# angelocatalani/neural-network-compression

Measured on AMD Instinct MI355X. Metric: weights/sec through prune+k-means (K=256), higher is better.
Workload: dtype f32

## Files before the change

### neural_network_compression_amd/csrc/nnc_hip.hip

```cpp
#include "nnc_common.hpp"
#include "nnc_km_shared.hpp"


extern "C" size_t nnc_kmeans_workspace_bytes(int32_t k)
{
    (void)k;
    return sizeof(KmWs) + 256;
}

extern "C" int32_t nnc_fix_shift(float absmax, int64_t n_total)
{
    int L = 1;
    while (((int64_t)1 << L) < n_total && L < 62) L++;
    if (!(absmax > 0.0f) || !std::isfinite(absmax)) return 0;
    int P = 0;
    (void)std::frexp((double)absmax, &P);
    return std::min(28, 62 - L) - P;
}

__device__ __forceinline__ int fix_f32(float v, int Sft)
{
    return (int)rintf(ldexpf(v, Sft));
}

// ... 1097 lines not shown
    return *word;
}

template <int NT, bool MASS>
__device__ int km_finalize_relocate(KmWs *__restrict__ ws, const float *__restrict__ xs, const long long n, const KmTab *__restrict__ tab, const int ku,
                                    const int k, const int cur, long long *sum_o, long long *cnt_o, const float mean, const int Sft)
{
    constexpr int KC = NNC_KMAX;
    __shared__ __align__(16) unsigned char buf[sizeof(KlHead) + (size_t)KC * (8 + 8 + 4 + 4 + 4 + 4 + 2 + 2) + 4096 * 2];
    KlHead *hd = reinterpret_cast<KlHead *>(buf);
    KlArr L = {};
    {
        unsigned char *q = buf + sizeof(KlHead);
        L.A = reinterpret_cast<long long *>(q); q += (size_t)KC * 8;
        L.B = reinterpret_cast<long long *>(q); q += (size_t)KC * 8;
        L.cs = reinterpret_cast<float *>(q); q += (size_t)KC * 4;
        L.csq = reinterpret_cast<float *>(q); q += (size_t)KC * 4;
        L.cold = reinterpret_cast<float *>(q); q += (size_t)KC * 4;
        L.call = reinterpret_cast<float *>(q); q += (size_t)KC * 4;
        L.so = reinterpret_cast<uint16_t *>(q); q += (size_t)KC * 2;
        L.phi = reinterpret_cast<uint16_t *>(q); q += (size_t)KC * 2;
        L.qj = reinterpret_cast<uint16_t *>(q);
    }
    const int tid = threadIdx.x;
    if (tid == 0) { hd->n_empty = 0; hd->ku = ku; hd->nch = 0; hd->slow = 0; hd->r_flat = 0; }
    __syncthreads();
    int e = 0;
    for (int j = tid; j < k; j += NT) { e += cnt_o[j] == 0; L.cold[j] = ws->c[cur][j]; }
    if (e) atomicAdd(&hd->n_empty, e);
    __syncthreads();
    const bool mass = MASS && hd->n_empty > KL_RM_MAX;
    if (!MASS && hd->n_empty > KL_RM_MAX) return 0;
    if (!mass && 2 * ku > KL_RPASS * (NT / 8)) return 0;
    for (int p = tid; p < ku; p += NT) {
        const float2 c = tab->cand[p];
        L.cs[p] = c.x; L.csq[p] = c.y; L.so[p] = tab->orig[p];
        L.A[p] = ws->hint_a[p]; L.B[p] = ws->hint_b[p];
        const int ph = ws->bnd_phi[p];
        L.phi[p] = (uint16_t)(ph < p + 1 ? p + 1 : (ph > ku - 1 ? ku - 1 : ph));
    }
    __syncthreads();
    int *qfirst = reinterpret_cast<int *>(L.call);
    for (int j = tid; j + 1 < ku; j += NT) {
        const long long bm = j > 0 ? L.B[j - 1] : 0, a = L.A[j], b = L.B[j];
        const long long s0 = a > bm ? a : bm;
        const long long len = b - s0;
        qfirst[j] = 0;
        if (len > 0) {
            const int cs_ = (int)L.phi[j] == j + 1 ? KL_CHUNK : KL_CHUNK_CROWD;
            const long long nc = (len + cs_ - 1) / cs_;
            if (nc > (mass ? 512 : 64)) hd->slow = 1;
            else {
                const int first = atomicAdd(&hd->nch, (int)nc);
                qfirst[j] = first;
                for (int i = 0; i < (int)nc; i++) if (first + i < KL_QMAX) L.qj[first + i] = (uint16_t)j;
            }
        }
    }
    __syncthreads();
    if (NNC_FIN_TRACE_PTR && tid == 0) {
        unsigned long long *rt = NNC_FIN_TRACE_PTR;
        const int it = min(ws->st.iter, 63);
        rt[300 + 4 * it] = (unsigned long long)hd->n_empty; rt[301 + 4 * it] = (unsigned long long)hd->nch; rt[302 + 4 * it] = (unsigned long long)hd->slow; rt[303 + 4 * it] = (unsigned long long)ku;
    }
    if (hd->slow || hd->nch > 1024) return 0;
    if constexpr (MASS) {
        if (mass) {
            __shared__ KlMass mass_s;
            return kl_relocate_mass<NT>(xs, n, ws, hd, L, &mass_s, sum_o, cnt_o, k, hd->nch, mean, Sft);
        }
    }
    return kl_relocate<NT>(xs, n, ws, hd, L, sum_o, cnt_o, k, hd->nch, mean, Sft);
}

template <int NT, bool ONEWAVE, bool MASS = false>
__device__ __forceinline__ bool km_finalize_body(KmWs *__restrict__ ws, int mode, int resume, int *gcell, int *hcell, int *ku_out, const bool lazy = false,
                                                 const float *__restrict__ reloc_xs = nullptr, const long long reloc_n = 0, const int k_hint = 0)
{
    static_assert(!ONEWAVE || NT == 64, "the barrier-free form is for a single wave");
#define FIN_SYNC() do { if (ONEWAVE) wave_lds_fence(); else km_lds_barrier(); } while (0)
#define FIN_OR(slot, x) (ONEWAVE ? (int)__any(x) : km_vote_or(&fin_votes[slot], (x)))
#define FIN_AND(slot, x) (ONEWAVE ? (int)__all(x) : !km_vote_or(&fin_votes[slot], !(x)))
#define FIN_COUNT(slot, x) (ONEWAVE ? (int)__popcll(__ballot(x)) : km_vote_count(&fin_votes[slot], (x)))
    __shared__ int fin_votes[8];
    __shared__ long long sum_o[NNC_KMAX];
    __shared__ long long cnt_o[NNC_KMAX];
    __shared__ __align__(16) float cnew[NNC_KMAX];
    __shared__ float cs[NNC_KMAX];
    __shared__ uint16_t so[NNC_KMAX];
    __shared__ float sq[NNC_KMAX];
    __shared__ unsigned long long sh_key;
    __shared__ int ovf_n;
    __shared__ PwHeap heap;
    __shared__ float cu[NNC_KMAX];
    __shared__ uint16_t sou[NNC_KMAX];
    __shared__ double wave_a[NT / 64], wave_b[NT / 64];

    const int tid = threadIdx.x;
    unsigned long long *ftr = NNC_FIN_TRACE_PTR;
#define FSTAMP(i) do { if (ftr && tid == 0) ftr[i] = __builtin_amdgcn_s_memrealtime(); } while (0)
    FSTAMP(0);
    if (tid == 0) ws->cells_pending = 0;
    if (!ONEWAVE && tid < 8) fin_votes[tid] = 0;
    const int kb = k_hint > 0 ? min(k_hint, (int)NNC_KMAX) : (int)NNC_KMAX;
    const bool takes_a_pass = mode != FIN_FROM_PARTIALS;
    const bool from_shards = mode == FIN_FROM_SHARDS || mode == FIN_PACK_ONLY;
    const int qn_raw = takes_a_pass ? ws->q_n : 0;
    const int st_done = ws->st.done, st_paused = ws->st.paused, st_iter = ws->st.iter, reloc_fail = ws->reloc_fail;
    const int spec_go = ws->spec_go;
    const int k = ws->p.k, Sft = ws->p.fix_shift, max_iter = ws->p.max_iter, glog2 = ws->glog2;
    const float tol_v = ws->p.tol, p_lo = ws->p.lo, p_hi = ws->p.hi, inv_f = ws->inv;
    const long long n_tot = ws->p.n_total;
    const int ku0 = ws->tab[0].ku, ku1 = ws->tab[1].ku;
    int cur = ws->cur;
    const bool track = (mode == FIN_FROM_SHARDS) || (mode == FIN_FROM_PARTIALS && !resume);
    constexpr int RR = 2;
    long long pc[RR];
    float c_both[RR][2];
    uint16_t pm_both[RR][2], pmn_both[RR][2];
#pragma unroll
    for (int r = 0; r < RR; r++) {
        pc[r] = 0; c_both[r][0] = c_both[r][1] = 0.0f; pm_both[r][0] = pm_both[r][1] = pmn_both[r][0] = pmn_both[r][1] = 0;
        const int j = tid + r * NT;
        if (j < kb) {
            if (track) pc[r] = ws->prev_counts[j];
            if (mode != FIN_INIT) {
                c_both[r][0] = ws->c[0][j]; c_both[r][1] = ws->c[1][j];
                pm_both[r][0] = ws->tab[0].perm[j]; pm_both[r][1] = ws->tab[1].perm[j];
                if (j + 1 < NNC_KMAX) { pmn_both[r][0] = ws->tab[0].perm[j + 1]; pmn_both[r][1] = ws->tab[1].perm[j + 1]; }
            }
        }
    }
    long long sh_s[KM_NSHARD];
    unsigned long long sh_c[KM_NSHARD];
    uint16_t og_both[2] = {0, 0};
    const bool sh_pre = from_shards && tid < kb;
#pragma unroll
    for (int sh = 0; sh < KM_NSHARD; sh++) { sh_s[sh] = 0; sh_c[sh] = 0; }
    if (sh_pre) {
        og_both[0] = ws->tab[0].orig[tid]; og_both[1] = ws->tab[1].orig[tid];
#pragma unroll
        for (int sh = 0; sh < KM_NSHARD; sh++) { sh_s[sh] = ws->shard_sum[sh][tid]; sh_c[sh] = ws->shard_cnt[sh][tid]; }
    }
    const int qn = min(qn_raw, (int)NNC_KMAX);
    for (int r = tid; r < qn; r += NT) { ws->q_w0[r] = 0ull; ws->q_w1[r] = 0ull; ws->q_next[r] = 0; }
    FSTAMP(44);
#define FIN_QUEUE_RESET() do { if (tid == 0 && takes_a_pass) { ws->q_n = 0; ws->q_searched = 0; ws->help_hint = qn > 0; } } while (0)
#define FIN_LEAVE() do { if (ONEWAVE) wave_lds_fence(); else __syncthreads(); FIN_QUEUE_RESET(); return false; } while (0)
    if (mode != FIN_INIT && mode != FIN_PACK_ONLY && st_done) FIN_LEAVE();
    if (mode == FIN_FROM_SHARDS && st_paused) FIN_LEAVE();
    if (mode == FIN_PACK_ONLY && (st_done | st_paused)) {
        const int k2 = 2 * k;
        for (int i = tid; i < k2; i += NT) ws->partials[i] = ws->partials_local[i];
        FIN_LEAVE();
    }
    if (mode == FIN_FROM_PARTIALS && st_paused && !resume) FIN_LEAVE();
    if (resume == 2 && !spec_go) FIN_LEAVE();
    if (resume && reloc_fail) {
        if (tid == 0) ws->st.paused = 2;
        FIN_LEAVE();
    }

    float cold_r[RR];
    int spa[RR], spb[RR];
#pragma unroll
    for (int r = 0; r < RR; r++) {
        const int j = tid + r * NT;
        const bool in = mode != FIN_INIT && j < k;
        cold_r[r] = in ? (cur ? c_both[r][1] : c_both[r][0]) : 0.0f;
        spa[r] = in ? (int)(cur ? pm_both[r][1] : pm_both[r][0]) : 0;
        spb[r] = (in && j + 1 < k) ? (int)(cur ? pmn_both[r][1] : pmn_both[r][0]) : 0;
        if (!(track && j < k)) pc[r] = 0;
    }
    if (from_shards) {
        const KmTab *tab = &ws->tab[cur];
        const int ku_cur = cur ? ku1 : ku0;
        for (int j = tid; j < k; j += NT) { sum_o[j] = 0; cnt_o[j] = 0; }
        FIN_SYNC();
        FIN_QUEUE_RESET();
        FSTAMP(45);
        for (int p = tid; p < ku_cur; p += NT) {
            long long s = 0;
            unsigned long long c = 0;
            int o;
            if (p == tid && sh_pre) {
                o = cur ? og_both[1] : og_both[0];
#pragma unroll
                for (int sh = 0; sh < KM_NSHARD; sh++) { s += sh_s[sh]; c += sh_c[sh]; }
            } else {
                o = tab->orig[p];
                for (int sh = 0; sh < KM_NSHARD; sh++) { s += ws->shard_sum[sh][p]; c += ws->shard_cnt[sh][p]; }
            }
            for (int sh = 0; sh < KM_NSHARD; sh++) { ws->shard_sum[sh][p] = 0; ws->shard_cnt[sh][p] = 0; }
            sum_o[o] = s; cnt_o[o] = (long long)c;
        }
        FIN_SYNC();
        FSTAMP(46);
        for (int j = tid; j < k; j += NT) {
            ws->partials[j] = sum_o[j]; ws->partials[k + j] = cnt_o[j];
            ws->partials_local[j] = sum_o[j]; ws->partials_local[k + j] = cnt_o[j];
        }
        if (mode == FIN_PACK_ONLY) return false;
    } else if (mode == FIN_FROM_PARTIALS) {
        for (int j = tid; j < k; j += NT) { sum_o[j] = ws->partials[j]; cnt_o[j] = ws->partials[k + j]; }
    }
    FIN_SYNC();
    FSTAMP(47);
    if (!from_shards) FIN_QUEUE_RESET();
    int same_counts_now = 0;
    bool settled_event = false;
    if (track) {
        int count_diff = 0;
#pragma unroll
        for (int r = 0; r < RR; r++) {
            const int j = tid + r * NT;
            if (j < k) {
                const long long c = cnt_o[j];
                count_diff |= (pc[r] != c);
                ws->prev_counts[j] = c;
            }
        }
        const int any_diff = FIN_OR(0, count_diff);
        same_counts_now = any_diff ? 0 : 1;
        if (tid == 0) ws->st.same_counts = any_diff ? 0 : 1;
    }
    FSTAMP(1);

    if (mode != FIN_INIT) {
        int my_empty = 0;
        for (int j = tid; j < k; j += NT) my_empty += (cnt_o[j] == 0);
        if (tid == 0) sh_key = 0ull;
        int n_empty = FIN_COUNT(1, my_empty);
        bool settled = false;
        settled_event = false;
        if constexpr (!ONEWAVE) {
            if (n_empty > 0 && (MASS || n_empty <= KL_RM_MAX) && !resume && reloc_xs && mode == FIN_FROM_SHARDS && lazy && !(st_iter >= 1 && same_counts_now)) {
                __syncthreads();
                if (ftr && tid == 0) { ftr[20] = ftr[0]; ftr[21] = __builtin_amdgcn_s_memrealtime(); }
                const KmTab *tabc = &ws->tab[cur];
                settled = km_finalize_relocate<NT, MASS>(ws, reloc_xs, reloc_n, tabc, cur ? ku1 : ku0, k, cur, sum_o, cnt_o, ws->p.x_mean, Sft) != 0;
                if (settled) { n_empty = 0; settled_event = true; }
                if (settled && ftr && tid == 0) ftr[22] = __builtin_amdgcn_s_memrealtime();
            }
        }
        if (n_empty > 0 && !resume) {
            int tot_empty = 0;
            if (tid == 0) {
                for (int j = 0; j < k; j++) tot_empty += (cnt_o[j] == 0);
                ws->st.paused = 1; ws->st.n_empty = tot_empty;
                if (lazy) ws->tab[cur].n_ovf = 0;
            }
            return false;
        }
        for (int j = tid; j < k; j += NT)
            if (cnt_o[j] > 0) cnew[j] = (float)ldexp((double)sum_o[j] / (double)cnt_o[j], -Sft);
        FIN_SYNC();
        if (n_empty > 0) {
            for (int j = tid; j < k; j += NT)
                atomicMax(&sh_key, ((unsigned long long)cnt_o[j] << 11) | (unsigned long long)(2047 - j));
            FIN_SYNC();
            const int amax = 2047 - (int)(sh_key & 2047ull);
            for (int j = tid; j < k; j += NT)
                if (cnt_o[j] <= 0) {
                    cnew[j] = (amax < j) ? cnew[amax] : (float)ldexp((double)sum_o[amax], -Sft);
                }
            FIN_SYNC();
        }
        FSTAMP(2);
#pragma unroll
        for (int r = 0; r < RR; r++) {
            const int j = tid + r * NT;
            if (j < k) {
                float d = cnew[j] - cold_r[r];
                float s2 = d * d;
                float sft = (float)sqrt((double)s2);
                sq[j] = sft * sft;
            }
        }
        FIN_SYNC();
        float tot = 0.0f;
        if (ONEWAVE) tot = block_pairwise_sum<true>([&](int i) { return sq[i]; }, k, &heap);
        else if (tid < 64) tot = wave_pairwise_sum([&](int i) { return sq[i]; }, k, &heap);
        if (tid == 0) {
            int iter = st_iter + 1;
            int done = 0;
            if (tot <= tol_v) done = 1;
            else if (iter >= max_iter) done = 2;
            ws->st.iter = iter; ws->st.shift_tot = tot; ws->st.done = done;
            ws->st.paused = 0; ws->st.n_empty = 0;
            ws->cur = cur ^ 1;
        }
        cur ^= 1;
        for (int j = tid; j < k; j += NT) ws->c[cur][j] = cnew[j];
        FIN_SYNC();
    } else {
        for (int j = tid; j < k; j += NT) cnew[j] = ws->c[cur][j];
        FIN_SYNC();
    }

    FSTAMP(3);
    KmTab *tab = &ws->tab[cur];
    int still_sorted = 0;
    if (mode != FIN_INIT) {
        int ok = 1;
#pragma unroll
        for (int r = 0; r < RR; r++) {
            const int p = tid + r * NT;
            if (p < k) {
                const int a = spa[r];
                so[p] = (uint16_t)a;
                cs[p] = cnew[a];
                if (p + 1 < k) {
                    const int b = spb[r];
                    const float va = cnew[a], vb = cnew[b];
                    ok &= (va < vb) || (va == vb && a < b);
                }
            }
        }
        FSTAMP(12);
        still_sorted = FIN_AND(2, ok);
        const bool moved_far = resume || settled_event;
        for (int pass = 0; pass < 3 && !still_sorted && !moved_far; pass++) {
            for (int parity = 0; parity < 2; parity++) {
                for (int p = 2 * tid + parity; p + 1 < k; p += 2 * NT) {
                    const float va = cs[p], vb = cs[p + 1];
                    const uint16_t a = so[p], b = so[p + 1];
                    if (!((va < vb) || (va == vb && a < b))) { cs[p] = vb; cs[p + 1] = va; so[p] = b; so[p + 1] = a; }
                }
                FIN_SYNC();
            }
            int ok2 = 1;
            for (int p = tid; p + 1 < k; p += NT) {
                const float va = cs[p], vb = cs[p + 1];
                ok2 &= (va < vb) || (va == vb && so[p] < so[p + 1]);
            }
            still_sorted = FIN_AND(3 + pass, ok2);
        }
    }
    FSTAMP(8);
    if (ftr && tid == 0) ftr[13] = (unsigned long long)still_sorted;
    if (!still_sorted) {
        int parts = 1;
        while (parts < 64 && k * parts * 2 <= NT) parts <<= 1;
        const int per_part = (((k + parts - 1) / parts) + 3) & ~3;
        const float4 *c4 = reinterpret_cast<const float4 *>(cnew);
        for (int t = tid; t < ((k * parts + NT - 1) / NT) * NT; t += NT) {
            const int j = t / parts, part = t % parts;
            int rank = 0;
            float v = 0.0f;
            if (j < k) {
                v = cnew[j];
                const int i0 = part * per_part, i1 = min(k, i0 + per_part);
#pragma unroll 4
                for (int i = i0; i < i1; i += 4) {
                    const float4 u = c4[i >> 2];
                    rank += (int)(u.x < v) | ((int)(u.x == v) & (int)(i < j));
                    rank += ((int)(u.y < v) | ((int)(u.y == v) & (int)(i + 1 < j))) & (int)(i + 1 < i1);
                    rank += ((int)(u.z < v) | ((int)(u.z == v) & (int)(i + 2 < j))) & (int)(i + 2 < i1);
                    rank += ((int)(u.w < v) | ((int)(u.w == v) & (int)(i + 3 < j))) & (int)(i + 3 < i1);
                }
            }
            for (int off = 1; off < parts; off <<= 1) rank += __shfl_xor(rank, off);
            if (j < k && part == 0) { cs[rank] = v; so[rank] = (uint16_t)j; }
        }
    }
    FIN_SYNC();
    FSTAMP(9);
    if (settled_event && ftr && tid == 0) { ftr[23] = ftr[3]; ftr[24] = ftr[9]; }
    int ku = 0;
    {
        int *wave_i = reinterpret_cast<int *>(wave_a);
        const int rounds_u = (k + NT - 1) / NT;
        int carry = 0;
        for (int rd = 0; rd < rounds_u; rd++) {
            const int p = rd * NT + tid;
            float v = 0.0f;
            int o = 0, first = 0;
            if (p < k) {
                v = cs[p]; o = so[p];
                tab->perm[p] = (uint16_t)o;
                first = (p == 0) || (cs[p - 1] != v);
            }
            const unsigned long long bal = __ballot(first);
            const int before = __popcll(bal & ((1ull << (tid & 63)) - 1ull));
            if ((tid & 63) == 0) wave_i[tid >> 6] = __popcll(bal);
            FIN_SYNC();
            int pre = carry, tot = carry;
            for (int w = 0; w < NT / 64; w++) { const int wv = wave_i[w]; if (w < (tid >> 6)) pre += wv; tot += wv; }
            if (first) { cu[pre + before] = v; sou[pre + before] = (uint16_t)o; }
            carry = tot;
            FIN_SYNC();
        }
        ku = min(carry, k);
    }
    FSTAMP(10);
    for (int p = tid; p < ku; p += NT) {
        const float v = cu[p];
        cs[p] = v;
        tab->cand[p] = make_float2(v, v * v);
        tab->orig[p] = sou[p];
        ws->bnd.cand[p] = make_float2(v, v * v);
        ws->bnd.orig[p] = sou[p];
    }
    if (tid == 0) { tab->ku = ku; ws->ku_cur = ku; ws->bnd.ku = ku; ovf_n = 0; }
    FIN_SYNC();
    FSTAMP(4);
    const double U = 5.9604644775390625e-08;
    const double xb = fmax(fabs((double)p_lo), fabs((double)p_hi));
    const int G = 1 << glog2;
    const double lo = (double)p_lo;
    const double inv = (double)inv_f;
    const double ra = inv > 0.0 ? (1.0 - 4.0 * U) / inv * (1.0 - 4.0 * U) : 0.0;
    const double rb = inv > 0.0 ? (1.0 + 4.0 * U) / inv * (1.0 + 4.0 * U) : 0.0;
    {
        const int rounds = (ku + NT - 1) / NT;
        int *wave_i = reinterpret_cast<int *>(wave_a);
        int carry_g = -2;
        int wide_zone = 0;
        double *zhi = reinterpret_cast<double *>(sum_o), *zlo = reinterpret_cast<double *>(cnt_o);
        const int zd = ku > 0 ? max(1, min(min(4, NT / max(ku, 1)), NNC_KMAX / max(ku, 1))) : 1;
        for (int t = tid; t < zd * ku; t += NT) {
            const int d = t / ku, p = t - d * ku, q = p + d + 1;
            if (q < ku) {
                const KmZone z = km_pair_zone((double)cs[p], (double)cs[q], xb);
                zhi[d * ku + p] = z.hi; zlo[d * ku + q] = z.lo;
            }
        }
        FSTAMP(13);
        FIN_SYNC();
        FSTAMP(14);
        for (int rd = 0; rd < rounds; rd++) {
            const int p = rd * NT + tid;
            int gp = -2, hp_ = G + 1;
            if (p < ku) {
                const double cp = (double)cs[p];
                double right = p + 1 < ku ? zhi[p] : INFINITY, left = p > 0 ? zlo[p] : -INFINITY;
                for (int q = p + 2; q < ku && q - p <= KM_ZONE_REACH; q++) {
                    const double cq = (double)cs[q];
                    const double mid = 0.5 * (cp + cq);
                    const double delta = cq - cp;
                    if (mid - km_pair_slack(delta, xb) >= right) break;
                    const int d = q - p - 1;
                    if (delta > 0.0) right = fmin(right, d < zd ? zhi[d * ku + p] : km_pair_zone(cp, cq, xb).hi);
                }
                for (int q = p - 2; q >= 0 && p - q <= KM_ZONE_REACH; q--) {
                    const double cq = (double)cs[q];
                    const double mid = 0.5 * (cp + cq);
                    const double delta = cp - cq;
                    if (mid + km_pair_slack(delta, xb) <= left) break;
                    const int d = p - q - 1;
                    if (delta > 0.0) left = fmax(left, d < zd ? zlo[d * ku + p] : km_pair_zone(cq, cp, xb).lo);
// ... 1910 lines not shown
```

### neural_network_compression_amd/csrc/nnc_lloyd.hpp

```cpp

struct KlDiag { unsigned long long ph[16], last, sp[8], slast; };
#ifdef NNC_DIAG
#define KLSTAMP(slot) do { if (threadIdx.x == 0) { const unsigned long long now_ = __builtin_amdgcn_s_memrealtime(); dg->ph[slot] += now_ - dg->last; dg->last = now_; } } while (0)
#define KLSUB(slot) do { if (threadIdx.x == 0) { const unsigned long long now_ = __builtin_amdgcn_s_memrealtime(); dg->sp[slot] += now_ - dg->slast; dg->slast = now_; } } while (0)
#else
#define KLSTAMP(slot) do { } while (0)
#define KLSUB(slot) do { } while (0)
#endif
#define KL_MAXR 24
#define KL_TAIL_MAX 2048

struct KlHeap { int start[64]; int len[64]; float val[64]; };
struct KlHead {
    int ku, slow, nch, n_empty, depth, pad0, pad1, pad2;
    float tot;
    int f_empty, f_diff, f_reorder;
    int wave_i[16];
    double wmax[16], wmin[16];
    KlHeap heap;
    int r_cnt, r_bad, r_flat, r_pad1;
    unsigned long long r_keys[8];
    unsigned long long r_wkey[2][16];
    int r_widx[2][16];
    int r_empty[8], r_old[8];
};
static_assert(sizeof(KlHead) % 16 == 0, "the arrays behind the header are 16-byte aligned");

struct KlArr {
    double *Lb, *Ub;
    long long *sum_s, *cnt_s, *A, *B, *PA, *PB, *prevc, *hint;
    float *hL, *hR, *cs, *csq, *cnew, *cold, *sq, *call, *Lf, *Uf;
    uint16_t *so, *perm, *phi, *qj;
};

static size_t kl_lds_bytes(int kc) { return sizeof(KlHead) + (size_t)kc * (2 * 8 + 9 * 8 + 12 * 4 + 3 * 2) + 4096 * 2; }

__device__ __forceinline__ void kl_carve(unsigned char *smem, int kc, KlHead **hd, KlArr *L)
{
    *hd = reinterpret_cast<KlHead *>(smem);
    unsigned char *p = smem + sizeof(KlHead);
    auto take = [&](size_t bytes) { unsigned char *q = p; p += bytes; return q; };
    L->Lb = reinterpret_cast<double *>(take((size_t)kc * 8)); L->Ub = reinterpret_cast<double *>(take((size_t)kc * 8));
    L->sum_s = reinterpret_cast<long long *>(take((size_t)kc * 8)); L->cnt_s = reinterpret_cast<long long *>(take((size_t)kc * 8));
    L->A = reinterpret_cast<long long *>(take((size_t)kc * 8)); L->B = reinterpret_cast<long long *>(take((size_t)kc * 8));
    L->PA = reinterpret_cast<long long *>(take((size_t)kc * 8)); L->PB = reinterpret_cast<long long *>(take((size_t)kc * 8));
    L->prevc = reinterpret_cast<long long *>(take((size_t)kc * 8)); L->hint = reinterpret_cast<long long *>(take((size_t)kc * 16));
    L->hL = reinterpret_cast<float *>(take((size_t)kc * 8)); L->hR = reinterpret_cast<float *>(take((size_t)kc * 8));
    L->cs = reinterpret_cast<float *>(take((size_t)kc * 4)); L->csq = reinterpret_cast<float *>(take((size_t)kc * 4));
    L->cnew = reinterpret_cast<float *>(take((size_t)kc * 4)); L->cold = reinterpret_cast<float *>(take((size_t)kc * 4));
    L->sq = reinterpret_cast<float *>(take((size_t)kc * 4)); L->call = reinterpret_cast<float *>(take((size_t)kc * 4));
    L->Lf = reinterpret_cast<float *>(take((size_t)kc * 4)); L->Uf = reinterpret_cast<float *>(take((size_t)kc * 4));
    L->so = reinterpret_cast<uint16_t *>(take((size_t)kc * 2)); L->perm = reinterpret_cast<uint16_t *>(take((size_t)kc * 2));
    L->phi = reinterpret_cast<uint16_t *>(take((size_t)kc * 2));
    L->qj = reinterpret_cast<uint16_t *>(take((size_t)4096 * 2));
}

#define KL_DPP_I(v, ctrl) __builtin_amdgcn_update_dpp(0, (v), (ctrl), 0xF, 0xF, true)
#define KL_QP_XOR1 0xB1
#define KL_QP_XOR2 0x4E
#define KL_HALF_MIRROR 0x141
__device__ __forceinline__ int grp8_sum_i(int v)
{
    v += KL_DPP_I(v, KL_QP_XOR1); v += KL_DPP_I(v, KL_QP_XOR2); v += KL_DPP_I(v, KL_HALF_MIRROR);
    return v;
}
__device__ __forceinline__ int grp8_min_i(int v)
{
    v = min(v, KL_DPP_I(v, KL_QP_XOR1)); v = min(v, KL_DPP_I(v, KL_QP_XOR2)); v = min(v, KL_DPP_I(v, KL_HALF_MIRROR));
    return v;
}
__device__ __forceinline__ long long grp8_sum_ll(long long v)
{
#define KL_STEP_LL(ctrl) do { const int lo_ = KL_DPP_I((int)(unsigned)(v & 0xFFFFFFFFll), ctrl), hi_ = KL_DPP_I((int)(v >> 32), ctrl); \
        v += (long long)(((unsigned long long)(unsigned)hi_ << 32) | (unsigned)lo_); } while (0)
    KL_STEP_LL(KL_QP_XOR1); KL_STEP_LL(KL_QP_XOR2); KL_STEP_LL(KL_HALF_MIRROR);
#undef KL_STEP_LL
    return v;
}

__device__ void kl_heap_build(KlHead *hd, int n)
{
    KlHeap *hp = &hd->heap;
    const int lane = threadIdx.x & 63;
    hp->start[lane] = 0; hp->len[lane] = 0; hp->val[lane] = 0.0f;
    wave_lds_fence();
    if (lane == 0) { hp->start[1] = 0; hp->len[1] = n; }
    wave_lds_fence();
    int depth = 0;
    while (depth < 5 && ((n + (1 << depth) - 1) >> depth) > LEAF) depth++;
    if (depth < 5) depth++;
    for (int lev = 0; lev < depth; lev++) {
        const int i = (1 << lev) + lane;
        if (lane < (1 << lev)) {
            const int l = hp->len[i];
            if (l > LEAF) {
                int n2 = l / 2; n2 -= n2 % 8;
                hp->start[2 * i] = hp->start[i]; hp->len[2 * i] = n2;
                hp->start[2 * i + 1] = hp->start[i] + n2; hp->len[2 * i + 1] = l - n2;
            }
        }
        wave_lds_fence();
    }
    if (lane == 0) hd->depth = depth;
}

__device__ __forceinline__ float kl_leaf_sum(const float *e, int st, int l, int j8)
{
// ... 427 lines not shown
            int best = j, besto = 0x7fffffff;
            for (int cc = j; cc <= (int)L.phi[j]; cc++) {
                const float d = L.csq[cc] + (-2.0f * (xc * L.cs[cc]));
                const int oc = (int)L.so[cc];
                if (d < bestd || (d == bestd && oc < besto)) { bestd = d; best = cc; besto = oc; }
            }
            atomicAdd(reinterpret_cast<unsigned long long *>(&L.sum_s[best]), (unsigned long long)((long long)fix_f32(xc, Sft) * len));
            atomicAdd(reinterpret_cast<unsigned long long *>(&L.cnt_s[best]), (unsigned long long)len);
            qfirst[j] = -1;
            hd->r_flat = 1;
        } else if (len > 0) {
            const int cs_ = (int)L.phi[j] == j + 1 ? KL_CHUNK : KL_CHUNK_CROWD;
            const long long nc = (len + cs_ - 1) / cs_;
            if (nc > KL_QONE) hd->slow = 1;
            else {
                const int first = atomicAdd(&hd->nch, (int)nc);
                qfirst[j] = first;
                for (int i = 0; i < (int)nc; i++) if (first + i < KL_QMAX) L.qj[first + i] = (uint16_t)j;
            }
        }
    }
}

template <int NT>
__device__ __forceinline__ void kl_label(const float *__restrict__ xs, const float mean, const int Sft, KlHead *hd, const KlArr &L)
{
    const int tid = threadIdx.x, g = tid >> 3, gl = tid & 7;
    const int nch = hd->nch;
    const int *qfirst = reinterpret_cast<const int *>(L.call);
    for (int c = g; c < nch; c += NT / 8) {
        const int j = (int)L.qj[c];
        const long long bm = j > 0 ? L.B[j - 1] : 0, a = L.A[j], e = L.B[j];
        const long long s = a > bm ? a : bm;
        const int phi = L.phi[j];
        const bool two = phi == j + 1;
        const int cs_ = two ? KL_CHUNK : KL_CHUNK_CROWD;
        const long long start = s + (long long)cs_ * (c - qfirst[j]);
        const long long end = start + cs_ < e ? start + cs_ : e;
        const float c0 = L.cs[j], q0 = L.csq[j], c1 = L.cs[j + 1], q1 = L.csq[j + 1];
        const bool tie1 = L.so[j + 1] < L.so[j];
        long long s0 = 0, s1 = 0;
        int n0 = 0, n1 = 0;
        for (long long r0 = start + gl; r0 < end; r0 += 64) {
            float v[8];
#pragma unroll
            for (int u = 0; u < 8; u++) { const long long r = r0 + 8 * u; v[u] = r < end ? xs[r] : 0.0f; }
#pragma unroll
            for (int u = 0; u < 8; u++) {
                if (r0 + 8 * u < end) {
                    const float xc = v[u] - mean;
                    const int q = fix_f32(xc, Sft);
                    if (two) {
                        const float d0 = q0 + (-2.0f * (xc * c0));
                        const float d1 = q1 + (-2.0f * (xc * c1));
                        if (d1 < d0 || (d1 == d0 && tie1)) { s1 += q; n1++; } else { s0 += q; n0++; }
                    } else {
                        float bestd = q0 + (-2.0f * (xc * c0));
                        int best = j, besto = (int)L.so[j];
                        for (int cc = j + 1; cc <= phi; cc++) {
                            const float d = L.csq[cc] + (-2.0f * (xc * L.cs[cc]));
                            const int oc = (int)L.so[cc];
                            if (d < bestd || (d == bestd && oc < besto)) { bestd = d; best = cc; besto = oc; }
                        }
                        atomicAdd(reinterpret_cast<unsigned long long *>(&L.sum_s[best]), (unsigned long long)(long long)q);
                        atomicAdd(reinterpret_cast<unsigned long long *>(&L.cnt_s[best]), 1ull);
                    }
                }
            }
        }
        const long long S0 = grp8_sum_ll(s0), S1 = grp8_sum_ll(s1);
        const int N01 = grp8_sum_i(n0 | (n1 << 16));
        if (gl == 0) {
            const int N0 = N01 & 0xFFFF, N1 = N01 >> 16;
            if (N0) { atomicAdd(reinterpret_cast<unsigned long long *>(&L.sum_s[j]), (unsigned long long)S0); atomicAdd(reinterpret_cast<unsigned long long *>(&L.cnt_s[j]), (unsigned long long)N0); }
            if (N1) { atomicAdd(reinterpret_cast<unsigned long long *>(&L.sum_s[j + 1]), (unsigned long long)S1); atomicAdd(reinterpret_cast<unsigned long long *>(&L.cnt_s[j + 1]), (unsigned long long)N1); }
        }
    }
}

#define KL_RW 8
#define KL_RM_MAX 7
#define KL_RKPT 16
#define KL_RPASS 10
template <int NT>
__device__ __forceinline__ int kl_relocate(const float *__restrict__ xs, const long long n, KmWs *__restrict__ ws, KlHead *hd, const KlArr &L,
                                           long long *sumo, long long *cnto, const int k, const int nch, const float mean, const int Sft)
{
    const int tid = threadIdx.x, lane = tid & 63, wv = tid >> 6, g = tid >> 3, gl = tid & 7;
    const int ku = hd->ku, m = hd->n_empty;
    if (tid == 0 && m > ws->kl_stats[7]) ws->kl_stats[7] = m;
    if (m < 1 || m > KL_RM_MAX || 2 * ku > KL_RPASS * (NT / 8) || hd->r_flat) { if (tid == 0) ws->kl_stats[6] |= 1; return 0; }
    unsigned long long *keys = ws->kl_keys;
    const int base = 2 * KL_RW * ku;
    unsigned long long *rtr = NNC_FIN_TRACE_PTR;
#define KRSTAMP(i) do { if (rtr && tid == 0) rtr[30 + (i)] = __builtin_amdgcn_s_memrealtime(); } while (0)
    KRSTAMP(0);
    if (tid == 0) { hd->r_cnt = 0; hd->r_bad = 0; }
    __syncthreads();
    unsigned inner = 0u;
    {
        long long rr[KL_RPASS];
        float xq[KL_RPASS];
        bool deep[KL_RPASS];
#pragma unroll
        for (int u = 0; u < KL_RPASS; u++) {
            const int q = g + u * (NT / 8);
            rr[u] = -1; deep[u] = false;
            if (q < 2 * ku) {
                const int p = q >> 1, side = q & 1;
                const long long lo_r = p > 0 ? L.B[p - 1] : 0, hi_r = p == ku - 1 ? n : L.A[p];
                long long r = -1;
                if (side == 0) { r = lo_r + gl; if (r >= hi_r) r = -1; }
                else { r = hi_r - 1 - gl; if (r < lo_r + KL_RW) r = -1; }
                rr[u] = r;
                deep[u] = gl == KL_RW - 1 && hi_r - lo_r > 2 * KL_RW;
            }
        }
#pragma unroll
        for (int u = 0; u < KL_RPASS; u++) xq[u] = rr[u] >= 0 ? xs[rr[u]] : 0.0f;
#pragma unroll
        for (int u = 0; u < KL_RPASS; u++) {
            const int q = g + u * (NT / 8);
            if (q < 2 * ku) {
                unsigned long long key = 0ull;
                if (rr[u] >= 0) {
                    const float dd = (xq[u] - mean) - L.cs[q >> 1];
                    const float dv = dd * dd;
                    key = ((unsigned long long)__float_as_uint(dv) << 32) | (unsigned long long)f32_ordered_bits(xq[u]);
                    if (deep[u]) inner = max(inner, __float_as_uint(dv));
                }
                keys[q * KL_RW + gl] = key;
            }
        }
    }
    KRSTAMP(1);
    const int *qfirst = reinterpret_cast<const int *>(L.call);
    for (int c = g; c < nch; c += NT / 8) {
        const int j = (int)L.qj[c];
        const long long bm = j > 0 ? L.B[j - 1] : 0, a = L.A[j], e = L.B[j];
        const long long s = a > bm ? a : bm;
        const int phi = L.phi[j];
        const int cs_ = phi == j + 1 ? KL_CHUNK : KL_CHUNK_CROWD;
        const long long start = s + (long long)cs_ * (c - qfirst[j]);
        const long long end = start + cs_ < e ? start + cs_ : e;
        int cbase = 0;
        if (gl == 0) cbase = atomicAdd(&hd->r_cnt, (int)(end - start));
        cbase = __shfl(cbase, (int)(threadIdx.x & 63 & ~7));
        for (long long r0 = start + gl; r0 < end; r0 += 64) {
            float xq[8];
#pragma unroll
            for (int u = 0; u < 8; u++) { const long long r = r0 + 8 * u; xq[u] = r < end ? xs[r] : 0.0f; }
#pragma unroll
            for (int u = 0; u < 8; u++) {
                if (r0 + 8 * u < end) {
                    const float xv = xq[u];
                    const float xc = xv - mean;
                    float bestd = L.csq[j] + (-2.0f * (xc * L.cs[j]));
                    int best = j, besto = (int)L.so[j];
                    for (int cc = j + 1; cc <= phi; cc++) {
                        const float d = L.csq[cc] + (-2.0f * (xc * L.cs[cc]));
                        const int oc = (int)L.so[cc];
                        if (d < bestd || (d == bestd && oc < besto)) { bestd = d; best = cc; besto = oc; }
                    }
                    const float dd = xc - L.cs[best];
                    const float dv = dd * dd;
                    const int slot = base + cbase + (int)(r0 + 8 * u - start);
                    if (slot < KL_RKEYS) keys[slot] = ((unsigned long long)__float_as_uint(dv) << 32) | (unsigned long long)f32_ordered_bits(xv);
                }
            }
        }
    }
    KRSTAMP(2);
    __syncthreads();
    KRSTAMP(3);
    const int N = base + hd->r_cnt;
    if (N > KL_RKPT * NT || N > KL_RKEYS) { if (tid == 0) ws->kl_stats[6] |= 2; return 0; }
    unsigned long long kr[KL_RKPT];
#pragma unroll
    for (int i = 0; i < KL_RKPT; i++) { const int slot = tid + i * NT; kr[i] = slot < N ? keys[slot] : 0ull; }
    KRSTAMP(4);
    if (tid <= KL_RM_MAX) hd->r_keys[tid] = 0ull;
#pragma unroll 1
    for (int r = 0; r <= m; r++) {
        {
            unsigned long long bk = 0ull;
            int bi = -1;
#pragma unroll
            for (int i = 0; i < KL_RKPT; i++) if (kr[i] > bk) { bk = kr[i]; bi = tid + i * NT; }
#pragma unroll
            for (int off = 32; off >= 1; off >>= 1) {
                const unsigned long long ok = (unsigned long long)__shfl_xor((long long)bk, off);
                const int oi = __shfl_xor(bi, off);
                if (ok > bk || (ok == bk && (unsigned)oi < (unsigned)bi)) { bk = ok; bi = oi; }
            }
            if (lane == 0) { hd->r_wkey[r & 1][wv] = bk; hd->r_widx[r & 1][wv] = bi; }
            __syncthreads();
            bk = 0ull; bi = -1;
#pragma unroll
            for (int w = 0; w < NT / 64; w++) {
                const unsigned long long ok = hd->r_wkey[r & 1][w];
                const int oi = hd->r_widx[r & 1][w];
                if (ok > bk || (ok == bk && (unsigned)oi < (unsigned)bi)) { bk = ok; bi = oi; }
            }
            if (tid == 0) hd->r_keys[r] = bk;
            if (bi >= 0 && (bi % NT) == tid) {
                const int mine = bi / NT;
#pragma unroll
                for (int i = 0; i < KL_RKPT; i++) if (i == mine) kr[i] = 0ull;
            }
        }
    }
    __syncthreads();
    KRSTAMP(5);
    const unsigned long long kcut = hd->r_keys[m - 1], ktop = hd->r_keys[0];
    int bad = 0;
    if (kcut == 0ull || (ktop >> 32) == 0ull) bad = 1;
    if (inner >= (unsigned)(kcut >> 32)) bad = 1;
    if (__syncthreads_or(bad)) { if (tid == 0) ws->kl_stats[6] |= (kcut == 0ull ? 4 : 0) | ((ktop >> 32) == 0ull ? 8 : 0) | 16; return 0; }
    {
        const int rounds = (k + NT - 1) / NT;
        int carry = 0;
        for (int rd = 0; rd < rounds; rd++) {
            const int j = rd * NT + tid;
            const int e = (j < k && cnto[j] == 0) ? 1 : 0;
            const unsigned long long bal = __ballot(e);
            const int before = __popcll(bal & ((1ull << lane) - 1ull));
            if (lane == 0) hd->wave_i[wv] = __popcll(bal);
            __syncthreads();
            int pre = carry, tot = carry;
            for (int w = 0; w < NT / 64; w++) { const int c = hd->wave_i[w]; if (w < wv) pre += c; tot += c; }
            if (e && pre + before < 8) hd->r_empty[pre + before] = j;
            carry = tot;
            __syncthreads();
        }
    }
    KRSTAMP(6);
    for (int i = wv; i < m; i += NT / 64) {
        const float xv = f32_from_ordered_bits((unsigned)(hd->r_keys[i] & 0xFFFFFFFFull));
        const float xc = xv - mean;
        float best = INFINITY;
        int old = 0x7fffffff;
        for (int j = lane; j < k; j += 64) {
            const float cv = L.cold[j];
            const float dj = cv * cv + (-2.0f * (xc * cv));
            if (dj < best) { best = dj; old = j; }
        }
#pragma unroll
        for (int off = 32; off >= 1; off >>= 1) {
            const float ob = __shfl_xor(best, off);
            const int oo = __shfl_xor(old, off);
            if (ob < best || (ob == best && oo < old)) { best = ob; old = oo; }
        }
        if (old == 0x7fffffff) old = 0;
        if (lane == 0) hd->r_old[i] = old;
    }
    __syncthreads();
    if (tid == 0) {
        int nb = 0;
        for (int i = 0; i < m; i++) {
            int leave = 0;
            for (int q = 0; q < m; q++) leave += hd->r_old[q] == hd->r_old[i];
            if (cnto[hd->r_old[i]] - leave < 1) nb = 1;
        }
        hd->r_bad = nb;
        if (nb) ws->kl_stats[6] |= 32;
        if (!nb) {
            for (int i = 0; i < m; i++) {
                const float xv = f32_from_ordered_bits((unsigned)(hd->r_keys[i] & 0xFFFFFFFFull));
                const long long v = (long long)fix_f32(xv - mean, Sft);
                const int old = hd->r_old[i], nw = hd->r_empty[i];
                sumo[old] -= v; cnto[old] -= 1;
                sumo[nw] += v; cnto[nw] += 1;
            }
            for (int i = 0; i < m; i++) {
                const int old = hd->r_old[i], nw = hd->r_empty[i];
                ws->partials[old] = sumo[old]; ws->partials[k + old] = cnto[old];
                ws->partials[nw] = sumo[nw]; ws->partials[k + nw] = cnto[nw];
            }
            if (m > 1) ws->st.reloc_multi += 1;
            const unsigned long long kn = hd->r_keys[m];
            if (kn != 0ull && (kn >> 32) == (kcut >> 32) && kn != kcut) ws->st.reloc_ties += 1;
            ws->st.n_relocated += 1;
            ws->st.n_in_place += 1;
            ws->reloc_fail = 0;
            ws->kl_stats[5] += 1;
        }
    }
    __syncthreads();
    KRSTAMP(7);
#undef KRSTAMP
    return hd->r_bad ? 0 : 1;
}

// ... 763 lines not shown
```

Baseline: 10.17 billion.

## Add bounded top-key selection in relocation and merge-based re-sort of moved centroids

The empty-cluster relocation path now first picks a per-wave top-(m+1) candidate threshold from boundary samples. It skips chunks whose distance bound cannot beat that threshold and gathers the few surviving keys for a single-wave select, which avoids the full block-wide key collection and multi-round reduction. When it cannot do this it falls back to the old path. The finalize step also adds a merge path: when only a minority of centroids came from previously empty clusters, it checks that the rest are still sorted and ranks the moved ones by counting and binary search instead of a full sort. Both add code, barriers and fallback branches, and they only help when their preconditions hold.

```diff
diff --git a/neural_network_compression_amd/csrc/nnc_hip.hip b/neural_network_compression_amd/csrc/nnc_hip.hip
--- a/neural_network_compression_amd/csrc/nnc_hip.hip
+++ b/neural_network_compression_amd/csrc/nnc_hip.hip
@@ -1203,6 +1203,7 @@
 #define FIN_OR(slot, x) (ONEWAVE ? (int)__any(x) : km_vote_or(&fin_votes[slot], (x)))
 #define FIN_AND(slot, x) (ONEWAVE ? (int)__all(x) : !km_vote_or(&fin_votes[slot], !(x)))
 #define FIN_COUNT(slot, x) (ONEWAVE ? (int)__popcll(__ballot(x)) : km_vote_count(&fin_votes[slot], (x)))
+    constexpr int RR = 2;
     __shared__ int fin_votes[8];
     __shared__ long long sum_o[NNC_KMAX];
     __shared__ long long cnt_o[NNC_KMAX];
@@ -1216,6 +1217,9 @@
     __shared__ float cu[NNC_KMAX];
     __shared__ uint16_t sou[NNC_KMAX];
     __shared__ double wave_a[NT / 64], wave_b[NT / 64];
+    uint16_t *was_empty = sou;
+    uint32_t *mv_o = reinterpret_cast<uint32_t *>(sq + NNC_KMAX / 2);
+    __shared__ int mv_cnt[RR * (NT / 64)];
 
     const int tid = threadIdx.x;
     unsigned long long *ftr = NNC_FIN_TRACE_PTR;
@@ -1235,7 +1239,6 @@
     const int ku0 = ws->tab[0].ku, ku1 = ws->tab[1].ku;
     int cur = ws->cur;
     const bool track = (mode == FIN_FROM_SHARDS) || (mode == FIN_FROM_PARTIALS && !resume);
-    constexpr int RR = 2;
     long long pc[RR];
     float c_both[RR][2];
     uint16_t pm_both[RR][2], pmn_both[RR][2];
@@ -1244,7 +1247,7 @@
         pc[r] = 0; c_both[r][0] = c_both[r][1] = 0.0f; pm_both[r][0] = pm_both[r][1] = pmn_both[r][0] = pmn_both[r][1] = 0;
         const int j = tid + r * NT;
         if (j < kb) {
-            if (track) pc[r] = ws->prev_counts[j];
+            if (track || resume) pc[r] = ws->prev_counts[j];
             if (mode != FIN_INIT) {
                 c_both[r][0] = ws->c[0][j]; c_both[r][1] = ws->c[1][j];
                 pm_both[r][0] = ws->tab[0].perm[j]; pm_both[r][1] = ws->tab[1].perm[j];
@@ -1291,7 +1294,7 @@
         cold_r[r] = in ? (cur ? c_both[r][1] : c_both[r][0]) : 0.0f;
         spa[r] = in ? (int)(cur ? pm_both[r][1] : pm_both[r][0]) : 0;
         spb[r] = (in && j + 1 < k) ? (int)(cur ? pmn_both[r][1] : pmn_both[r][0]) : 0;
-        if (!(track && j < k)) pc[r] = 0;
+        if (!((track || resume) && j < k)) pc[r] = 0;
     }
     if (from_shards) {
         const KmTab *tab = &ws->tab[cur];
@@ -1350,6 +1353,11 @@
     if (mode != FIN_INIT) {
         int my_empty = 0;
         for (int j = tid; j < k; j += NT) my_empty += (cnt_o[j] == 0);
+#pragma unroll
+        for (int r = 0; r < RR; r++) {
+            const int j = tid + r * NT;
+            if (j < k) was_empty[j] = (uint16_t)(resume ? pc[r] == 0 : cnt_o[j] == 0);
+        }
         if (tid == 0) sh_key = 0ull;
         int n_empty = FIN_COUNT(1, my_empty);
         bool settled = false;
@@ -1422,6 +1430,7 @@
     FSTAMP(3);
     KmTab *tab = &ws->tab[cur];
     int still_sorted = 0;
+    bool merged = false;
     if (mode != FIN_INIT) {
         int ok = 1;
 #pragma unroll
@@ -1457,10 +1466,79 @@
             }
             still_sorted = FIN_AND(3 + pass, ok2);
         }
+        if (!still_sorted && moved_far) {
+            constexpr int NW = NT / 64;
+            int fl[RR], before[RR];
+#pragma unroll
+            for (int r = 0; r < RR; r++) {
+                const int p = tid + r * NT;
+                fl[r] = p < k ? (int)was_empty[spa[r]] : 0;
+                const unsigned long long bal = __ballot(fl[r]);
+                before[r] = __popcll(bal & ((1ull << (tid & 63)) - 1ull));
+                if ((tid & 63) == 0) mv_cnt[r * NW + (tid >> 6)] = __popcll(bal);
+            }
+            FIN_SYNC();
+            int pre[RR], m = 0;
+#pragma unroll
+            for (int r = 0; r < RR; r++) {
+                pre[r] = m;
+                for (int w = 0; w < NW; w++) { const int c = mv_cnt[r * NW + w]; if (w < (tid >> 6)) pre[r] += c; m += c; }
+            }
+            if (m >= 1 && 2 * m <= k) {
+                const int nr = k - m;
+#pragma unroll
+                for (int r = 0; r < RR; r++) {
+                    const int p = tid + r * NT;
+                    if (p < k) {
+                        const int a = spa[r], mi = pre[r] + before[r];
+                        if (fl[r]) { sq[mi] = cnew[a]; mv_o[mi] = (uint32_t)a; }
+                        else { cu[p - mi] = cnew[a]; sou[p - mi] = (uint16_t)a; }
+                    }
+                }
+                FIN_SYNC();
+                int ok = 1;
+#pragma unroll
+                for (int r = 0; r < RR; r++) {
+                    const int q = tid + r * NT;
+                    if (q + 1 < nr) {
+                        const float va = cu[q], vb = cu[q + 1];
+                        ok &= (int)(va < vb) | ((int)(va == vb) & (int)(sou[q] < sou[q + 1]));
+                    }
+                }
+                if (FIN_AND(7, ok)) {
+                    merged = true;
+#pragma unroll
+                    for (int r = 0; r < RR; r++) {
+                        const int t = tid + r * NT;
+                        if (t < k) {
+                            const bool from_r = t < nr;
+                            const float v = from_r ? cu[t] : sq[t - nr];
+                            const int o = from_r ? (int)sou[t] : (int)mv_o[t - nr];
+                            int rank = 0;
+                            for (int i = 0; i < m; i++) {
+                                const float u = sq[i];
+                                rank += (int)(u < v) | ((int)(u == v) & (int)((int)mv_o[i] < o));
+                            }
+                            if (from_r) rank += t;
+                            else {
+                                int lo_ = 0, hi_ = nr;
+                                while (lo_ < hi_) {
+                                    const int mid = (lo_ + hi_) >> 1;
+                                    const float u = cu[mid];
+                                    if ((u < v) || (u == v && (int)sou[mid] < o)) lo_ = mid + 1; else hi_ = mid;
+                                }
+                                rank += lo_;
+                            }
+                            cs[rank] = v; so[rank] = (uint16_t)o;
+                        }
+                    }
+                }
+            }
+        }
     }
     FSTAMP(8);
     if (ftr && tid == 0) ftr[13] = (unsigned long long)still_sorted;
-    if (!still_sorted) {
+    if (!still_sorted && !merged) {
         int parts = 1;
         while (parts < 64 && k * parts * 2 <= NT) parts <<= 1;
         const int per_part = (((k + parts - 1) / parts) + 3) & ~3;
@@ -1488,6 +1566,20 @@
     FIN_SYNC();
     FSTAMP(9);
     if (settled_event && ftr && tid == 0) { ftr[23] = ftr[3]; ftr[24] = ftr[9]; }
+#ifdef NNC_DIAG
+    if (ftr && (resume || settled_event) && !still_sorted) {
+        int wrong = 0;
+        for (int p = tid; p < k && merged; p += NT) {
+            const float v = cs[p];
+            const int j = (int)so[p];
+            int rank = 0;
+            for (int i = 0; i < k; i++) { const float u = cnew[i]; rank += (int)(u < v) | ((int)(u == v) & (int)(i < j)); }
+            wrong += (rank != p) || (cnew[j] != v && !(cnew[j] != cnew[j]));
+        }
+        if (wrong) atomicAdd(&ftr[18], (unsigned long long)wrong);
+        if (tid == 0) atomicAdd(&ftr[merged ? 17 : 19], 1ull);
+    }
+#endif
     int ku = 0;
     {
         int *wave_i = reinterpret_cast<int *>(wave_a);
diff --git a/neural_network_compression_amd/csrc/nnc_lloyd.hpp b/neural_network_compression_amd/csrc/nnc_lloyd.hpp
--- a/neural_network_compression_amd/csrc/nnc_lloyd.hpp
+++ b/neural_network_compression_amd/csrc/nnc_lloyd.hpp
@@ -23,6 +23,9 @@
     unsigned long long r_wkey[2][16];
     int r_widx[2][16];
     int r_empty[8], r_old[8];
+    int r_ns, r_pad2[3];
+    unsigned long long r_top[16 * 8];
+    unsigned long long r_surv[128];
 };
 static_assert(sizeof(KlHead) % 16 == 0, "the arrays behind the header are 16-byte aligned");
 
@@ -616,6 +619,36 @@
 #define KL_RM_MAX 7
 #define KL_RKPT 16
 #define KL_RPASS 10
+#define KL_RSURV 128
+
+template <int NR>
+__device__ __forceinline__ unsigned long long kl_wave_select(unsigned long long (&kr)[NR], const int cnt, unsigned long long *out)
+{
+    const int lane = threadIdx.x & 63;
+    unsigned long long last = 0ull;
+#pragma unroll 1
+    for (int r = 0; r < cnt; r++) {
+        unsigned long long bk = 0ull;
+        int bi = -1;
+#pragma unroll
+        for (int i = 0; i < NR; i++) if (kr[i] > bk) { bk = kr[i]; bi = i * 64 + lane; }
+#pragma unroll
+        for (int off = 32; off >= 1; off >>= 1) {
+            const unsigned long long ok = (unsigned long long)__shfl_xor((long long)bk, off);
+            const int oi = __shfl_xor(bi, off);
+            if (ok > bk || (ok == bk && (unsigned)oi < (unsigned)bi)) { bk = ok; bi = oi; }
+        }
+        if (bi >= 0 && (bi & 63) == lane) {
+            const int mine = bi >> 6;
+#pragma unroll
+            for (int i = 0; i < NR; i++) if (i == mine) kr[i] = 0ull;
+        }
+        if (out && lane == 0) out[r] = bk;
+        last = bk;
+    }
+    return last;
+}
+
 template <int NT>
 __device__ __forceinline__ int kl_relocate(const float *__restrict__ xs, const long long n, KmWs *__restrict__ ws, KlHead *hd, const KlArr &L,
                                            long long *sumo, long long *cnto, const int k, const int nch, const float mean, const int Sft)
@@ -629,9 +662,134 @@
     unsigned long long *rtr = NNC_FIN_TRACE_PTR;
 #define KRSTAMP(i) do { if (rtr && tid == 0) rtr[30 + (i)] = __builtin_amdgcn_s_memrealtime(); } while (0)
     KRSTAMP(0);
+    unsigned inner = 0u;
+    const int *qfirst = reinterpret_cast<const int *>(L.call);
+    bool selected = false;
+    {
+        if (tid == 0) { hd->r_cnt = 0; hd->r_bad = 0; hd->r_ns = 0; }
+        if (tid <= KL_RM_MAX) hd->r_keys[tid] = 0ull;
+        km_lds_barrier();
+        unsigned long long ek[KL_RPASS], sk[KL_RPASS];
+        {
+            long long rr[KL_RPASS];
+            float xq[KL_RPASS];
+            bool deep[KL_RPASS];
+#pragma unroll
+            for (int u = 0; u < KL_RPASS; u++) {
+                const int q = g + u * (NT / 8);
+                rr[u] = -1; deep[u] = false;
+                if (q < 2 * ku) {
+                    const int p = q >> 1, side = q & 1;
+                    const long long lo_r = p > 0 ? L.B[p - 1] : 0, hi_r = p == ku - 1 ? n : L.A[p];
+                    long long r = -1;
+                    if (side == 0) { r = lo_r + gl; if (r >= hi_r) r = -1; }
+                    else { r = hi_r - 1 - gl; if (r < lo_r + KL_RW) r = -1; }
+                    rr[u] = r;
+                    deep[u] = gl == KL_RW - 1 && hi_r - lo_r > 2 * KL_RW;
+                }
+            }
+#pragma unroll
+            for (int u = 0; u < KL_RPASS; u++) xq[u] = rr[u] >= 0 ? xs[rr[u]] : 0.0f;
+            for (int c = g; c < nch; c += NT / 8) {
+                if (gl == 0) {
+                    const int j = (int)L.qj[c];
+                    const long long bm = j > 0 ? L.B[j - 1] : 0, a = L.A[j], e = L.B[j];
+                    const long long s = a > bm ? a : bm;
+                    const int cs_ = (int)L.phi[j] == j + 1 ? KL_CHUNK : KL_CHUNK_CROWD;
+                    const long long start = s + (long long)cs_ * (c - qfirst[j]);
+                    const long long end = start + cs_ < e ? start + cs_ : e;
+                    atomicAdd(&hd->r_cnt, (int)(end - start));
+                }
+            }
+#pragma unroll
+            for (int u = 0; u < KL_RPASS; u++) {
+                const int q = g + u * (NT / 8);
+                ek[u] = 0ull;
+                if (q < 2 * ku && rr[u] >= 0) {
+                    const float dd = (xq[u] - mean) - L.cs[q >> 1];
+                    const float dv = dd * dd;
+                    ek[u] = ((unsigned long long)__float_as_uint(dv) << 32) | (unsigned long long)f32_ordered_bits(xq[u]);
+                    if (deep[u]) inner = max(inner, __float_as_uint(dv));
+                }
+                sk[u] = gl == 0 ? ek[u] : 0ull;
+            }
+        }
+        kl_wave_select<KL_RPASS>(sk, m + 1, &hd->r_top[wv * (m + 1)]);
+        km_lds_barrier();
+        KRSTAMP(1);
+        const int N = base + hd->r_cnt;
+        if (N > KL_RKPT * NT || N > KL_RKEYS) { if (tid == 0) ws->kl_stats[6] |= 2; return 0; }
+        unsigned long long t2[2];
+#pragma unroll
+        for (int i = 0; i < 2; i++) { const int idx = lane + 64 * i; t2[i] = idx < (NT / 64) * (m + 1) ? hd->r_top[idx] : 0ull; }
+        const unsigned long long Lkey = kl_wave_select<2>(t2, m + 1, nullptr);
+        if (Lkey != 0ull) {
+            const unsigned Ld = (unsigned)(Lkey >> 32);
+#pragma unroll
+            for (int u = 0; u < KL_RPASS; u++)
+                if (ek[u] >= Lkey) { const int slot = atomicAdd(&hd->r_ns, 1); if (slot < KL_RSURV) hd->r_surv[slot] = ek[u]; }
+            for (int c = g; c < nch; c += NT / 8) {
+                const int j = (int)L.qj[c];
+                const long long bm = j > 0 ? L.B[j - 1] : 0, a = L.A[j], e = L.B[j];
+                const long long s = a > bm ? a : bm;
+                const int phi = L.phi[j];
+                const int cs_ = phi == j + 1 ? KL_CHUNK : KL_CHUNK_CROWD;
+                const long long start = s + (long long)cs_ * (c - qfirst[j]);
+                const long long end = start + cs_ < e ? start + cs_ : e;
+                if (end <= start) continue;
+                const float x0 = xs[start] - mean, x1 = xs[end - 1] - mean;
+                unsigned bound = 0u;
+                for (int cc = j; cc <= phi; cc++) {
+                    const float d0 = x0 - L.cs[cc], d1 = x1 - L.cs[cc];
+                    bound = max(bound, max(__float_as_uint(d0 * d0), __float_as_uint(d1 * d1)));
+                }
+                if (bound < Ld) continue;
+                for (long long r0 = start + gl; r0 < end; r0 += 64) {
+                    float xv8[8];
+#pragma unroll
+                    for (int u = 0; u < 8; u++) { const long long r = r0 + 8 * u; xv8[u] = r < end ? xs[r] : 0.0f; }
+#pragma unroll
+                    for (int u = 0; u < 8; u++) {
+                        if (r0 + 8 * u < end) {
+                            const float xv = xv8[u];
+                            const float xc = xv - mean;
+                            float bestd = L.csq[j] + (-2.0f * (xc * L.cs[j]));
+                            int best = j, besto = (int)L.so[j];
+                            for (int cc = j + 1; cc <= phi; cc++) {
+                                const float d = L.csq[cc] + (-2.0f * (xc * L.cs[cc]));
+                                const int oc = (int)L.so[cc];
+                                if (d < bestd || (d == bestd && oc < besto)) { bestd = d; best = cc; besto = oc; }
+                            }
+                            const float dd = xc - L.cs[best];
+                            const float dv = dd * dd;
+                            const unsigned long long key = ((unsigned long long)__float_as_uint(dv) << 32) | (unsigned long long)f32_ordered_bits(xv);
+                            if (key >= Lkey) { const int slot = atomicAdd(&hd->r_ns, 1); if (slot < KL_RSURV) hd->r_surv[slot] = key; }
+                        }
+                    }
+                }
+            }
+            KRSTAMP(2);
+            km_lds_barrier();
+            KRSTAMP(3);
+            KRSTAMP(4);
+            const int ns = hd->r_ns;
+            if (ns <= KL_RSURV) {
+                if (wv == 0) {
+                    unsigned long long sv[KL_RSURV / 64];
+#pragma unroll
+                    for (int i = 0; i < KL_RSURV / 64; i++) { const int idx = lane + 64 * i; sv[i] = idx < ns ? hd->r_surv[idx] : 0ull; }
+                    kl_wave_select<KL_RSURV / 64>(sv, m + 1, hd->r_keys);
+                }
+                selected = true;
+            }
+        }
+        if (tid == 0) ws->kl_stats[6] |= selected ? 64 : (Lkey == 0ull ? 128 : 256);
+    }
+    if (!selected) {
+    __syncthreads();
+    inner = 0u;
     if (tid == 0) { hd->r_cnt = 0; hd->r_bad = 0; }
     __syncthreads();
-    unsigned inner = 0u;
     {
         long long rr[KL_RPASS];
         float xq[KL_RPASS];
@@ -668,7 +826,6 @@
         }
     }
     KRSTAMP(1);
-    const int *qfirst = reinterpret_cast<const int *>(L.call);
     for (int c = g; c < nch; c += NT / 8) {
         const int j = (int)L.qj[c];
         const long long bm = j > 0 ? L.B[j - 1] : 0, a = L.A[j], e = L.B[j];
@@ -743,6 +900,7 @@
                 for (int i = 0; i < KL_RKPT; i++) if (i == mine) kr[i] = 0ull;
             }
         }
+    }
     }
     __syncthreads();
     KRSTAMP(5);
```

After: 9.856 billion. 0.969x the previous value.
